# ahuang73/HemoCell

Measured on AMD Instinct MI355X. Metric: MLUPS + cell-vertex updates/s, 256^3 pipeflow 10% Hct, higher is better.
Workload: dtype f64

## Files before the change

hemocell_amd/capi.py:

```python
import ctypes as C
import os
import subprocess

_HERE = os.path.dirname(os.path.abspath(__file__))
LIB_PATH = os.path.join(_HERE, "lib", "libhemocell_amd.so")

c_double_p = C.POINTER(C.c_double)
c_long_p = C.POINTER(C.c_long)
c_int_p = C.POINTER(C.c_int)


class HcError(RuntimeError):
    pass


class Params(C.Structure):
    _fields_ = [(n, C.c_double) for n in
                ("dx", "dt", "nu_p", "rho_p", "kBT_p", "tau", "nu_lbm", "dm", "df", "f_limit", "kBT_lbm")]


class Material(C.Structure):
    _fields_ = [("kLink", C.c_double), ("kArea", C.c_double), ("kVolume", C.c_double), ("kBend", C.c_double),
                ("eta_m", C.c_double), ("radius", C.c_double), ("min_triangles", C.c_int),
                ("aspect_ratio", C.c_double), ("inner_edges", c_long_p), ("n_inner", C.c_int)]


class WbcMaterial(C.Structure):
    _fields_ = [("kInnerRigid", C.c_double), ("kCytoskeleton", C.c_double), ("coreRadius", C.c_double),
                ("radius", C.c_double)]


class CellTypeSpec(C.Structure):
    _fields_ = [("model", C.c_int), ("shape", C.c_int), ("material", Material), ("wbc", C.POINTER(WbcMaterial)),
                ("kInnerLink", C.c_double), ("stl_path", C.c_char_p)]


VP = C.c_void_p
SIGNATURES = {
    "hc_last_error": (C.c_char_p, []),
    "hc_init": (C.c_int, [C.c_int]),
    "hc_device_count": (C.c_int, [c_int_p]),
    "hc_set_stream": (C.c_int, [VP]),
    "hc_synchronize": (C.c_int, []),
    "hc_fork": (C.c_int, []),
    "hc_route": (C.c_int, [C.c_int]),
    "hc_join": (C.c_int, []),
    "hc_side_stream": (C.c_int, [C.POINTER(VP)]),
    "hc_set_overlap": (C.c_int, [C.c_int]),
    "hc_comm_init_env": (C.c_int, []),
    "hc_comm_init": (C.c_int, [C.c_int, C.c_int, C.c_int, C.c_char_p, C.c_int, C.c_int, C.c_int]),
    "hc_comm_finalize": (C.c_int, []),
    "hc_comm_info": (C.c_int, [c_int_p, c_int_p, c_int_p]),
    "hc_comm_barrier": (C.c_int, []),
    "hc_comm_allreduce": (C.c_int, [c_double_p, C.c_int, C.c_int]),
    "hc_comm_bcast": (C.c_int, [VP, C.c_size_t, C.c_int]),
    "hc_comm_allgather": (C.c_int, [VP, C.c_size_t, VP]),
    "hc_comm_exchange_host": (C.c_int, [C.c_int, VP, C.c_size_t, VP, C.c_size_t, VP, C.c_size_t, VP, C.c_size_t]),
    "hc_slab_stats": (C.c_int, [VP, c_double_p, C.c_int]),
    "hcl_slab_refresh_halos": (C.c_int, [VP, C.c_int]),
    "hcp_slab_sync_placement": (C.c_int, [VP, c_long_p]),
    "hcp_set_envelope": (C.c_int, [VP, C.c_double, c_double_p]),
    "hcp_envelope": (C.c_int, [VP, c_double_p, c_long_p]),
    "hcp_set_deletion_mode": (C.c_int, [VP, C.c_int]),
    "hcp_delete_incomplete_cells": (C.c_int, [VP, c_long_p]),
    "hcp_deletion_counts": (C.c_int, [VP, c_long_p, c_long_p, c_long_p, c_long_p]),
    "hcp_download_alive": (C.c_int, [VP, VP]),
    "hc_profile_enable": (C.c_int, [C.c_int]),
    "hc_profile_read": (C.c_int, [C.c_char_p, c_double_p, c_long_p]),
    "hc_profile_reset": (C.c_int, []),
    "hc_build_tag": (C.c_char_p, []),
    "hc_measure_copy_bandwidth": (C.c_int, [C.c_size_t, C.c_int, c_double_p]),
    "hcl_node_counts": (C.c_int, [VP, c_long_p]),
    "hc_debug_ibm_per_vertex": (C.c_int, [C.c_int]),
    "hc_set_reproducible_spread": (C.c_int, [C.c_int]),
    "hc_debug_force_plane_padding": (C.c_int, [C.c_int]),
    "hcl_create": (C.c_int, [C.POINTER(VP), C.c_int, C.c_int, C.c_int, c_int_p, C.c_double, C.c_int, C.c_int, C.c_int]),
    "hcl_destroy": (C.c_int, [VP]),
    "hcl_set_mask": (C.c_int, [VP, VP]),
    "hcl_init_equilibrium": (C.c_int, [VP, C.c_double, c_double_p]),
    "hcl_set_body_force_regions": (C.c_int, [VP, C.c_int, C.POINTER(C.c_int), c_double_p]),
    "hcl_set_body_force": (C.c_int, [VP, c_double_p]),
    "hcl_set_wall_velocity": (C.c_int, [VP, C.c_int, c_double_p]),
    "hcl_collide_stream": (C.c_int, [VP, C.c_int]),
    "hcl_set_lees_edwards": (C.c_int, [VP, C.c_double, C.c_double]),
    "hcl_set_lees_edwards_displacement": (C.c_int, [VP, C.c_double, C.c_double]),
    "hcl_lees_edwards_apply": (C.c_int, [VP]),
    "hcl_lees_edwards_state": (C.c_int, [VP, c_double_p]),
    "hcl_open_boundary_add": (C.c_int, [VP, C.c_int, C.c_int, c_int_p, C.c_int, c_int_p]),
    "hcl_open_boundary_add_box": (C.c_int, [VP, C.c_int, C.c_int, c_int_p, c_int_p, c_int_p]),
    "hcl_open_boundary_add_axis": (C.c_int, [VP, C.c_int, C.c_int, C.c_int, c_int_p, C.c_int, c_int_p]),
    "hcl_open_boundary_add_box_axis": (C.c_int, [VP, C.c_int, C.c_int, C.c_int, c_int_p, c_int_p, c_int_p]),
    "hcl_open_boundary_axes": (C.c_int, [VP, c_int_p, C.c_int, c_int_p]),
    "hcl_open_boundary_clear": (C.c_int, [VP]),
    "hcl_open_boundary_slots": (C.c_int, [VP, c_int_p, C.c_int, c_int_p]),
    "hcl_open_boundary_set_velocity": (C.c_int, [VP, C.c_int, C.c_int, VP, C.c_int]),
    "hcl_open_boundary_set_density": (C.c_int, [VP, C.c_int, C.c_int, VP, C.c_int]),
    "hcl_open_boundary_values": (C.c_int, [VP, C.c_int, C.c_int, c_double_p]),
    "hcl_plane_velocity": (C.c_int, [VP, C.c_int, c_int_p, C.c_int, VP, C.c_int]),
    "hcl_collide_stream_part": (C.c_int, [VP, C.c_int]),
    "hcl_step_end": (C.c_int, [VP]),
    "hcl_download_populations": (C.c_int, [VP, c_double_p]),
    "hcl_upload_populations": (C.c_int, [VP, c_double_p]),
    "hcl_download_rho_u": (C.c_int, [VP, c_double_p, c_double_p]),
    "hcl_download_pi_neq": (C.c_int, [VP, c_double_p]),
    "hcl_download_ibm_force": (C.c_int, [VP, c_double_p]),
    "hcl_zero_ibm_force": (C.c_int, [VP]),
    "hcl_halo_doubles": (C.c_size_t, [VP, C.c_int]),
    "hcl_halo_pack": (C.c_int, [VP, C.c_int, C.c_int, VP]),
    "hcl_halo_unpack": (C.c_int, [VP, C.c_int, C.c_int, VP]),
    "hcl_halo_pack_next": (C.c_int, [VP, C.c_int, C.c_int, VP]),
    "hcl_face_velocity_pack": (C.c_int, [VP, C.c_int, VP]),
    "hcl_face_velocity_pack_both": (C.c_int, [VP, VP, VP]),
    "hcl_halo_pack_both": (C.c_int, [VP, VP, VP, C.c_int]),
    "hcl_halo_unpack_both": (C.c_int, [VP, VP, VP]),
    "hcl_zero_force_halos": (C.c_int, [VP]),
    "hcl_download_face_velocity": (C.c_int, [VP, C.c_int, c_double_p]),
    "hcl_dims": (C.c_int, [VP, c_int_p]),
    "hcl_mlups_bytes_per_node": (C.c_double, [VP]),
    "hc_params_base": (C.c_int, [C.POINTER(Params)] + [C.c_double] * 5),
    "hcp_celltype_create": (C.c_int, [C.POINTER(VP), C.c_int, C.c_int, C.POINTER(Params), C.POINTER(Material)]),
    "hcp_celltype_create_wbc": (C.c_int, [C.POINTER(VP), C.c_int, C.POINTER(Params), C.POINTER(Material),
                                          C.POINTER(WbcMaterial)]),
    "hcp_celltype_wbc_constants": (C.c_int, [VP, c_double_p]),
    "hcp_celltype_create_ex": (C.c_int, [C.POINTER(VP), C.POINTER(Params), C.POINTER(CellTypeSpec)]),
    "hcp_celltype_malaria_constants": (C.c_int, [VP, c_double_p]),
    "hcp_celltype_destroy": (C.c_int, [VP]),
    "hcp_celltype_sizes": (C.c_int, [VP, c_int_p]),
    "hcp_celltype_tables": (C.c_int, [VP, c_double_p, c_long_p, c_long_p, c_double_p, c_double_p, c_double_p,
                                      c_long_p, c_double_p, c_double_p]),
    "hcp_celltype_tables2": (C.c_int, [VP, c_long_p, c_long_p, c_long_p, c_double_p, c_int_p]),
    "hcp_create": (C.c_int, [C.POINTER(VP), VP, C.POINTER(Params)]),
    "hcp_destroy": (C.c_int, [VP]),
    "hcp_add_type": (C.c_int, [VP, VP, C.c_int, c_int_p]),
    "hcp_add_cell": (C.c_int, [VP, C.c_int, C.c_long, c_double_p, c_double_p, C.c_double, c_int_p]),
    "hcp_add_cell_unchecked": (C.c_int, [VP, C.c_int, C.c_long, c_double_p, c_double_p]),
    "hcp_counts": (C.c_int, [VP, c_long_p, c_long_p, c_long_p]),
    "hcp_type_range": (C.c_int, [VP, C.c_int, c_long_p, c_long_p]),
    "hcp_download": (C.c_int, [VP, C.c_int, c_double_p]),
    "hcp_upload": (C.c_int, [VP, C.c_int, c_double_p]),
    "hcp_download_cell_ids": (C.c_int, [VP, c_long_p]),
    "hcp_download_records": (C.c_int, [VP, C.c_void_p, C.c_long]),
    "hcp_upload_records": (C.c_int, [VP, C.c_void_p, C.c_long]),
    "hcp_add_vertex_force": (C.c_int, [VP, c_long_p, C.c_int, c_double_p]),
    "hcp_set_repulsion": (C.c_int, [VP, C.c_double, C.c_double, C.c_int]),
    "hcp_repulsion": (C.c_int, [VP]),
    "hcp_download_repulsion": (C.c_int, [VP, c_double_p]),
    "hcl_fluid_stats": (C.c_int, [VP, C.c_int, c_double_p, C.POINTER(C.c_long)]),
    "hcp_vertex_stats": (C.c_int, [VP, C.c_int, c_double_p, C.POINTER(C.c_long)]),
    "hcp_set_boundary_repulsion": (C.c_int, [VP, C.c_double, C.c_double, C.c_int]),
    "hcp_boundary_repulsion": (C.c_int, [VP]),
    "hcp_spread": (C.c_int, [VP, C.c_int]),
    "hcp_interpolate": (C.c_int, [VP]),
    "hcp_interpolate_cells": (C.c_int, [VP, C.c_int, c_int_p, C.c_int]),
    "hcp_advance": (C.c_int, [VP, C.c_int]),
    "hcp_mechanics": (C.c_int, [VP, C.c_long, C.c_int]),
    "hcp_mechanics_components": (C.c_int, [VP, C.c_int, c_double_p]),
    "hc_iterate": (C.c_int, [VP, VP, c_long_p, C.c_int, C.c_int, C.c_int, C.c_int]),
    "hcp_cell_extents": (C.c_int, [VP, C.c_int, c_double_p]),
# ... 44 lines not shown
```

hemocell_amd/csrc/lattice.hip:

```cpp
#include "common.h"
#include "comm.h"
#include <algorithm>
#include <type_traits>

using namespace hc;

namespace {

struct LatArgs {
  const double *fin;
  double *fout;
  const double *Fin;
  double *Fzero;
  const uint8_t *mask;
  int nx, ny, nz;
  int plane;
  long xs;
  long npad;
  long qs;
  int x_begin;
  int x_split, x_jump;
  int wrap_x, per_y, per_z;
  double omega;
  double bx, by, bz;
  const int *row_z0, *row_cum, *blk_row;
  int nblk;
  int ibm;
  const uint8_t *dirty_in, *dirty_zero; uint8_t epoch_in, epoch_zero;
  double wall_u[4][3];
  int x0, nx_global;
  BodyRegions reg;
};

struct OpenArgs : LatArgs {
  const int *ob_code;
  const double *ob_val;
};
template <bool OPEN> using Args = std::conditional_t<OPEN, OpenArgs, LatArgs>;

__device__ __forceinline__ void body_at(const LatArgs &a, int x, int y, int z, double &bx, double &by, double &bz) {
  bx = a.bx; by = a.by; bz = a.bz;
  if (a.reg.n) region_force(a.reg, a.x0 + x, y, z, bx, by, bz);
}

struct Nbr {
  long xm, xp;
  int ym, yp, zm, zp;
  bool ym_ok, yp_ok, zm_ok, zp_ok;
};

__device__ __forceinline__ Nbr neighbours(const LatArgs &a, int x, int y, int z) {
  Nbr n;
  n.xm = -a.xs; n.xp = a.xs;
  if (a.wrap_x) {
    if (x == 0) n.xm = (long)(a.nx - 1) * a.xs;
    if (x == a.nx - 1) n.xp = -(long)(a.nx - 1) * a.xs;
  }
  n.ym = -a.nz; n.yp = a.nz; n.ym_ok = n.yp_ok = true;
  if (y == 0) { if (a.per_y) n.ym = (a.ny - 1) * a.nz; else n.ym_ok = false; }
  if (y == a.ny - 1) { if (a.per_y) n.yp = -(a.ny - 1) * a.nz; else n.yp_ok = false; }
  n.zm = -1; n.zp = 1; n.zm_ok = n.zp_ok = true;
  if (z == 0) { if (a.per_z) n.zm = a.nz - 1; else n.zm_ok = false; }
  if (z == a.nz - 1) { if (a.per_z) n.zp = -(a.nz - 1); else n.zp_ok = false; }
  return n;
}

template <int CX, int CY, int CZ>
__device__ __forceinline__ long src_off(const Nbr &n, bool &ok) {
  long off = 0; ok = true;
  if (CX == 1) off += n.xm; else if (CX == -1) off += n.xp;
  if (CY == 1) { off += n.ym; ok = ok && n.ym_ok; } else if (CY == -1) { off += n.yp; ok = ok && n.yp_ok; }
  if (CZ == 1) { off += n.zm; ok = ok && n.zm_ok; } else if (CZ == -1) { off += n.zp; ok = ok && n.zp_ok; }
  return off;
}
template <int CX, int CY, int CZ>
__device__ __forceinline__ long dst_off(const Nbr &n, bool &ok) {
  long off = 0; ok = true;
  if (CX == 1) off += n.xp; else if (CX == -1) off += n.xm;
  if (CY == 1) { off += n.yp; ok = ok && n.yp_ok; } else if (CY == -1) { off += n.ym; ok = ok && n.ym_ok; }
  if (CZ == 1) { off += n.zp; ok = ok && n.zp_ok; } else if (CZ == -1) { off += n.zm; ok = ok && n.zm_ok; }
  return off;
}

#define FOR_Q(M)                                                                                     \
  M(0, 0, 0, 0) M(1, -1, 0, 0) M(2, 0, -1, 0) M(3, 0, 0, -1) M(4, -1, -1, 0) M(5, -1, 1, 0)          \
  M(6, -1, 0, -1) M(7, -1, 0, 1) M(8, 0, -1, -1) M(9, 0, -1, 1) M(10, 1, 0, 0) M(11, 0, 1, 0)        \
  M(12, 0, 0, 1) M(13, 1, 1, 0) M(14, 1, -1, 0) M(15, 1, 0, 1) M(16, 1, 0, -1) M(17, 0, 1, 1)        \
  M(18, 0, 1, -1)

__device__ __forceinline__ constexpr double tq(int q) { return q == 0 ? 1. / 3. : ((q >= 1 && q <= 3) || (q >= 10 && q <= 12)) ? 1. / 18. : 1. / 36.; }

__device__ __forceinline__ void pull(const double *__restrict__ fin, long npad, long node, const Nbr &n, double f[HC_Q]) {
#define M(Q, CX, CY, CZ)                                   \
  {                                                        \
    bool ok; long off = src_off<CX, CY, CZ>(n, ok);        \
    f[Q] = ok ? fin[(long)Q * npad + node + off] : 0.0;    \
  }
  FOR_Q(M)
#undef M
}

template <bool OPEN>
__device__ __forceinline__ void complete_open(const Args<OPEN> &a, long node, double f[HC_Q]) {
  if constexpr (OPEN) {
    if (a.mask[node] == 0) {
      const int code = a.ob_code[node];
      if (code >= 0) zou_he_node(f, code, a.ob_val);
    }
  }
}

__device__ __forceinline__ void moments(const double f[HC_Q], double &rhoBar, double &jx, double &jy, double &jz) {
  double r = 0.0, x = 0.0, y = 0.0, z = 0.0;
#define M(Q, CX, CY, CZ)              \
  r += f[Q];                          \
  if (CX == 1) x += f[Q]; else if (CX == -1) x += -f[Q]; \
  if (CY == 1) y += f[Q]; else if (CY == -1) y += -f[Q]; \
  if (CZ == 1) z += f[Q]; else if (CZ == -1) z += -f[Q];
  FOR_Q(M)
#undef M
  rhoBar = r; jx = x; jy = y; jz = z;
}

template <int CX, int CY, int CZ>
__device__ __forceinline__ double cdot(double a0, double a1, double a2) {
  double s = 0.0; bool first = true;
  if (CX != 0) { s = (CX == 1 ? a0 : -a0); first = false; }
  if (CY != 0) { double t = (CY == 1 ? a1 : -a1); s = first ? t : s + t; first = false; }
  if (CZ != 0) { double t = (CZ == 1 ? a2 : -a2); s = first ? t : s + t; first = false; }
  return s;
}

__device__ __forceinline__ void collide_guo(double f[HC_Q], double Fx, double Fy, double Fz, double omega) {
  double rhoBar, j0, j1, j2;
  moments(f, rhoBar, j0, j1, j2);
  const double invRho = 1.0 / (1.0 + rhoBar);
  const double rho = 1.0 + rhoBar;
  const double u0 = j0 * invRho + Fx / 2.0, u1 = j1 * invRho + Fy / 2.0, u2 = j2 * invRho + Fz / 2.0;
  j0 = rho * u0; j1 = rho * u1; j2 = rho * u2;
  const double jSqr = j0 * j0 + j1 * j1 + j2 * j2;
  const double one_m_omega = 1.0 - omega;
  const double guo = 1.0 - omega / 2.0;
#define M(Q, CX, CY, CZ)                                                                     \
  {                                                                                          \
    const double c_j = cdot<CX, CY, CZ>(j0, j1, j2);                                         \
    const double feq = tq(Q) * (rhoBar + 3.0 * c_j + invRho * (4.5 * c_j * c_j - 1.5 * jSqr)); \
    f[Q] *= one_m_omega;                                                                     \
    f[Q] += omega * feq;                                                                     \
  }
  FOR_Q(M)
#undef M
#define M(Q, CX, CY, CZ)                                                                     \
  {                                                                                          \
    double c_u = cdot<CX, CY, CZ>(u0, u1, u2);                                               \
    c_u *= 9.0;                                                                              \
    double ft = (((double)CX - u0) * 3.0 + c_u * (double)CX) * Fx;                           \
    ft += (((double)CY - u1) * 3.0 + c_u * (double)CY) * Fy;                                 \
    ft += (((double)CZ - u2) * 3.0 + c_u * (double)CZ) * Fz;                                 \
    ft *= tq(Q);                                                                             \
    ft *= guo;                                                                               \
    f[Q] += ft;                                                                              \
  }
  FOR_Q(M)
#undef M
}

template <bool REGIONS, bool OPEN = false>
__global__ __launch_bounds__(256) void collide_stream_kernel(Args<OPEN> a) {
  const int x = a.x_begin + (int)blockIdx.y + ((int)blockIdx.y >= a.x_split ? a.x_jump : 0);
  const int xp = x + HALO;
  const int t = blockIdx.x * 256 + threadIdx.x;
  const int *cum = a.row_cum + (long)xp * (a.ny + 1);
  if (t >= cum[a.ny]) return;
  int lo = a.blk_row[(long)xp * (a.nblk + 1) + blockIdx.x], hi = a.blk_row[(long)xp * (a.nblk + 1) + blockIdx.x + 1];
  while (lo < hi) { const int mid = (lo + hi + 1) >> 1; if (cum[mid] <= t) lo = mid; else hi = mid - 1; }
  const int y = lo, z = a.row_z0[(long)xp * a.ny + y] + (t - cum[y]);
  const int p = y * a.nz + z;
  const long node = (long)(x + HALO) * a.xs + p;
  const uint8_t m = a.mask[node];
  if (m == 2) return;
  const Nbr n = neighbours(a, x, y, z);
  const bool fdirty = a.ibm && m == 0 && a.dirty_in[node >> 4] == a.epoch_in;
  double F0 = 0.0, F1 = 0.0, F2 = 0.0;
  if (fdirty) { F0 = a.Fin[3 * node]; F1 = a.Fin[3 * node + 1]; F2 = a.Fin[3 * node + 2]; }
  double f[HC_Q];
  pull(a.fin, a.qs, node, n, f);
  const bool wall = m != 0;
  if (wall) {
#pragma unroll
    for (int i = 1; i <= 9; i++) { double t = f[i]; f[i] = f[i + 9]; f[i + 9] = t; }
    if (m >= 3) {
      const double w0 = a.wall_u[m - 3][0], w1 = a.wall_u[m - 3][1], w2 = a.wall_u[m - 3][2];
#define M(Q, CX, CY, CZ)                                                                  \
      if (Q != 0) {                                                                       \
        constexpr int O = Q <= 9 ? Q + 9 : Q - 9;                                         \
        const double c_u = (double)CX * w0 + (double)CY * w1 + (double)CZ * w2;           \
        f[O] = f[O] - 6.0 * tq(Q) * c_u;                                                  \
      }
      FOR_Q(M)
#undef M
    }
  } else {
    double bx = a.bx, by = a.by, bz = a.bz;
    if (REGIONS) region_force(a.reg, a.x0 + x, y, z, bx, by, bz);
    double Fx = bx, Fy = by, Fz = bz;
    if (fdirty) {
      Fx = bx + F0; Fy = by + F1; Fz = bz + F2;
    }
    if constexpr (OPEN) {
      const int code = a.ob_code[node];
      if (code >= 0) zou_he_node(f, code, a.ob_val);
    }
    collide_guo(f, Fx, Fy, Fz, a.omega);
  }
#pragma unroll
  for (int q = 0; q < HC_Q; q++) __builtin_nontemporal_store(f[q], &a.fout[(long)q * a.qs + node]);
  if (a.ibm && a.dirty_zero[node >> 4] == a.epoch_zero) { a.Fzero[3 * node] = 0.0; a.Fzero[3 * node + 1] = 0.0; a.Fzero[3 * node + 2] = 0.0; }
}

__global__ void init_eq_kernel(LatArgs a, double rhoBar, double j0, double j1, double j2) {
  const int p = blockIdx.x * 256 + threadIdx.x;
  if (p >= a.plane) return;
  const int x = a.x_begin + blockIdx.y;
  const int y = p / a.nz, z = p - y * a.nz;
  const long node = (long)(x + HALO) * a.xs + p;
  const Nbr n = neighbours(a, x, y, z);
  const double invRho = 1.0 / (1.0 + rhoBar);
  const double jSqr = j0 * j0 + j1 * j1 + j2 * j2;
#define M(Q, CX, CY, CZ)                                                                        \
  {                                                                                             \
    bool ok; long off = dst_off<CX, CY, CZ>(n, ok);                                             \
    double v = 0.0;                                                                             \
    if (ok && a.mask[node + off] == 0) {                                                        \
      const double c_j = cdot<CX, CY, CZ>(j0, j1, j2);                                          \
      v = tq(Q) * (rhoBar + 3.0 * c_j + invRho * (4.5 * c_j * c_j - 1.5 * jSqr));               \
    }                                                                                           \
    a.fout[(long)Q * a.qs + node] = v;                                                          \
  }
  FOR_Q(M)
#undef M
}

__global__ void download_kernel(LatArgs a, double *aos) {
  const int p = blockIdx.x * 256 + threadIdx.x;
  if (p >= a.plane) return;
  const int x = a.x_begin + blockIdx.y;
  const int y = p / a.nz, z = p - y * a.nz;
  const long node = (long)(x + HALO) * a.xs + p;
  const Nbr n = neighbours(a, x, y, z);
  double f[HC_Q];
  pull(a.fin, a.qs, node, n, f);
  const long o = ((long)x * a.plane + p) * HC_Q;
#pragma unroll
  for (int q = 0; q < HC_Q; q++) aos[o + q] = f[q];
}

__global__ void upload_kernel(LatArgs a, const double *aos, int lo_ok, int hi_ok) {
  const int p = blockIdx.x * 256 + threadIdx.x;
  if (p >= a.plane) return;
  const int x = a.x_begin + blockIdx.y;
  const int y = p / a.nz, z = p - y * a.nz;
  const long node = (long)(x + HALO) * a.xs + p;
  const long bulk = (long)x * a.plane + p;
  Nbr nl = neighbours(a, x, y, z);
  nl.xm = nl.xm / a.xs * a.plane; nl.xp = nl.xp / a.xs * a.plane;
#define M(Q, CX, CY, CZ)                                                                  \
  {                                                                                       \
    bool ok; long off = dst_off<CX, CY, CZ>(nl, ok);                                      \
     \
    if (!a.wrap_x && ((CX == 1 && x == a.nx - 1 && !hi_ok) || (CX == -1 && x == 0 && !lo_ok))) ok = false; \
    a.fout[(long)Q * a.qs + node] = ok ? aos[(bulk + off) * HC_Q + Q] : 0.0;            \
  }
  FOR_Q(M)
#undef M
}

template <bool OPEN = false>
__global__ void rho_u_kernel(Args<OPEN> a, double *rho, double *u) {
  const int p = blockIdx.x * 256 + threadIdx.x;
  if (p >= a.plane) return;
  const int x = a.x_begin + blockIdx.y;
  const int y = p / a.nz, z = p - y * a.nz;
  const long node = (long)(x + HALO) * a.xs + p;
  const Nbr n = neighbours(a, x, y, z);
  double f[HC_Q];
  pull(a.fin, a.qs, node, n, f);
  complete_open<OPEN>(a, node, f);
  double rhoBar, j0, j1, j2;
  moments(f, rhoBar, j0, j1, j2);
  const double invRho = 1.0 / (1.0 + rhoBar);
  const long o = (long)x * a.plane + p;
  rho[o] = 1.0 + rhoBar;
  double bx, by, bz;
  body_at(a, x, y, z, bx, by, bz);
  u[3 * o] = j0 * invRho + (bx + a.Fin[3 * node]) / 2.0;
  u[3 * o + 1] = j1 * invRho + (by + a.Fin[3 * node + 1]) / 2.0;
  u[3 * o + 2] = j2 * invRho + (bz + a.Fin[3 * node + 2]) / 2.0;
}

template <bool OPEN = false>
// ... 144 lines not shown
  const long s2 = top ? modp((long)floor(D + (double)x), a.nx) : modp((long)ceil(-D + (double)x), a.nx);
  double f1[HC_Q], f2[HC_Q];
  pull(a.fin, a.qs, (s1 + HALO) * a.xs + row, neighbours(a, (int)s1, y, z), f1);
  pull(a.fin, a.qs, (s2 + HALO) * a.xs + row, neighbours(a, (int)s2, y, z), f2);
  if (top) {
    f[3] = g * f1[3] + (1 - g) * f2[3];
    f[6] = g * f1[16] + (1 - g) * f2[16];
    f[8] = g * f1[8] + (1 - g) * f2[8];
    f[16] = g * f1[6] + (1 - g) * f2[6];
    f[18] = g * f1[18] + (1 - g) * f2[18];
  } else {
    f[7] = g * f1[15] + (1 - g) * f2[15];
    f[9] = g * f1[9] + (1 - g) * f2[9];
    f[12] = g * f1[12] + (1 - g) * f2[12];
    f[15] = g * f1[7] + (1 - g) * f2[7];
    f[17] = g * f1[17] + (1 - g) * f2[17];
  }
  double *o = buf + (long)(1 - top) * HC_Q * nxy + r;
#pragma unroll
  for (int q = 0; q < HC_Q; q++) o[(long)q * nxy] = f[q];
}

__global__ __launch_bounds__(256) void le_scatter_kernel(LatArgs a, const double *buf) {
  const long nxy = (long)a.nx * a.ny;
  const long t = (long)blockIdx.x * 256 + threadIdx.x;
  if (t >= 2 * nxy) return;
  const int top = t < nxy ? 1 : 0;
  const long r = top ? t : t - nxy;
  const int x = (int)(r / a.ny), y = (int)(r - (long)x * a.ny);
  const int z = top ? a.nz - 1 : 0;
  const long node = (long)(x + HALO) * a.xs + (long)y * a.nz + z;
  const Nbr n = neighbours(a, x, y, z);
  const double *in = buf + (long)(1 - top) * HC_Q * nxy + r;
#define M(Q, CX, CY, CZ)                                                       \
  {                                                                            \
    bool ok; const long off = src_off<CX, CY, CZ>(n, ok);                      \
    if (ok) a.fout[(long)Q * a.qs + node + off] = in[(long)Q * nxy];           \
  }
  FOR_Q(M)
#undef M
}

struct HaloArgs {
  double *f;
  double *buf;
  double *buf2; int n_first;
  long npad; long xs; int plane;
  int n;
  int pop[HC_Q + 5];
  int xp[HC_Q + 5];
  int to_buf;
};
__global__ void halo_copy_kernel(HaloArgs h) {
  const int p = blockIdx.x * 256 + threadIdx.x;
  if (p >= h.plane) return;
  const int e = blockIdx.y;
  const long li = (long)h.pop[e] * h.npad + (long)h.xp[e] * h.xs + p;
  double *b = e < h.n_first ? h.buf + (long)e * h.plane + p : h.buf2 + (long)(e - h.n_first) * h.plane + p;
  if (h.to_buf) *b = h.f[li]; else h.f[li] = *b;
}

__global__ void zero_force_halo_kernel(double *F, long xs, int plane, int nx) {
  const int e = blockIdx.x * 256 + threadIdx.x;
  if (e >= 3 * plane) return;
  const int w = blockIdx.y;
  const int xp = w < HALO ? w : nx + w;
  F[3 * (long)xp * xs + e] = 0.0;
}

LatArgs make_args(const hc_lattice *L) {
  LatArgs a;
  a.fin = L->f[L->cur]; a.fout = L->f[1 - L->cur];
  const int fprev = (L->fcur + 2) % 3;
  a.Fin = L->force[L->fcur]; a.Fzero = L->force[fprev];
  a.x_split = 0x7fffffff; a.x_jump = 0;
  a.mask = L->mask;
  a.nx = L->nx; a.ny = L->ny; a.nz = L->nz; a.plane = (int)L->plane; a.xs = (long)L->xs; a.npad = (long)L->npad; a.qs = (long)L->qstride;
  a.x_begin = 0;
  a.wrap_x = (L->n_slabs == 1 && L->periodic[0]) ? 1 : 0;
  a.per_y = L->periodic[1]; a.per_z = L->periodic[2];
  a.omega = L->omega; a.bx = L->body[0]; a.by = L->body[1]; a.bz = L->body[2];
  a.x0 = L->x0; a.nx_global = L->nx_global; a.reg = L->regions;
  a.row_z0 = L->row_z0; a.row_cum = L->row_cum; a.blk_row = L->blk_row; a.nblk = L->nblk;
  a.ibm = L->ibm;
  a.dirty_in = L->fdirty[L->fcur]; a.dirty_zero = L->fdirty[fprev]; a.epoch_in = L->fepoch[L->fcur]; a.epoch_zero = L->fepoch[fprev];
  for (int c = 0; c < 4; c++) for (int d = 0; d < 3; d++) a.wall_u[c][d] = L->wall_u[c][d];
  return a;
}

OpenArgs open_args(const hc_lattice *L, const LatArgs &a) {
  OpenArgs o;
  static_cast<LatArgs &>(o) = a;
  o.ob_code = L->ob_code; o.ob_val = L->ob_val;
  return o;
}

dim3 plane_grid(const hc_lattice *L, int nplanes) { return dim3((unsigned)((L->plane + 255) / 256), (unsigned)nplanes, 1); }

int ensure_scratch(hc_lattice *L, size_t doubles) {
  if (L->scratch_doubles >= doubles) return HC_OK;
  if (L->scratch) HC_HIP(hipFree(L->scratch));
  L->scratch = nullptr; L->scratch_doubles = 0;
  HC_HIP(hipMalloc((void **)&L->scratch, doubles * sizeof(double)));
  L->scratch_doubles = doubles;
  return HC_OK;
}

int rebuild_active_map(hc_lattice *L) {
  const int NX = L->nx + 2 * HALO, ny = L->ny, nz = L->nz;
  std::vector<int> z0((size_t)NX * ny), cum((size_t)NX * (ny + 1));
  int max_active = 0;
  for (int x = 0; x < NX; x++) {
    int c = 0;
    for (int y = 0; y < ny; y++) {
      const uint8_t *row = L->hmask.data() + (size_t)x * L->xs + (size_t)y * nz;
      int a = 0, b = nz;
      while (a < nz && row[a] == 2) a++;
      while (b > a && row[b - 1] == 2) b--;
      z0[(size_t)x * ny + y] = a;
      cum[(size_t)x * (ny + 1) + y] = c;
      c += b - a;
    }
    cum[(size_t)x * (ny + 1) + ny] = c;
    max_active = std::max(max_active, c);
  }
  if (max_active == 0) max_active = 1;
  const int nblk = (max_active + 255) / 256;
  std::vector<int> blk((size_t)NX * (nblk + 1));
  for (int x = 0; x < NX; x++) {
    const int *cx = cum.data() + (size_t)x * (ny + 1);
    int y = 0;
    for (int b = 0; b <= nblk; b++) {
      const long t = (long)b * 256;
      while (y + 1 < ny && cx[y + 1] <= t) y++;
      blk[(size_t)x * (nblk + 1) + b] = y;
    }
  }
  for (int **p : {&L->row_z0, &L->row_cum, &L->blk_row}) if (*p) { HC_HIP(hipFree(*p)); *p = nullptr; }
  HC_HIP(hipMalloc((void **)&L->row_z0, z0.size() * sizeof(int)));
  HC_HIP(hipMalloc((void **)&L->row_cum, cum.size() * sizeof(int)));
  HC_HIP(hipMalloc((void **)&L->blk_row, blk.size() * sizeof(int)));
  HC_HIP(hipMemcpy(L->row_z0, z0.data(), z0.size() * sizeof(int), hipMemcpyHostToDevice));
  HC_HIP(hipMemcpy(L->row_cum, cum.data(), cum.size() * sizeof(int), hipMemcpyHostToDevice));
  HC_HIP(hipMemcpy(L->blk_row, blk.data(), blk.size() * sizeof(int), hipMemcpyHostToDevice));
  L->nblk = nblk; L->max_active = max_active;
  return HC_OK;
}

int rebuild_wall_bricks(hc_lattice *L) {
  const int NX = L->nx + 2 * HALO, ny = L->ny, nz = L->nz;
  std::vector<uint8_t> flag((size_t)L->nbx * L->nby * L->nbz, 0);
  for (int bx = 0; bx < L->nbx; bx++)
    for (int by = 0; by < L->nby; by++)
      for (int bz = 0; bz < L->nbz; bz++) {
        bool near = false;
        if (!L->periodic[1] && (by == 0 || by == L->nby - 1)) near = true;
        if (!L->periodic[2] && (bz == 0 || bz == L->nbz - 1)) near = true;
        if (bx * 8 < HALO + 1 || bx * 8 + 7 >= L->nx + HALO - 1) near = true;
        for (int x = bx * 8; x < std::min(NX, bx * 8 + 8) && !near; x++)
          for (int y = by * 8; y < std::min(ny, by * 8 + 8) && !near; y++) {
            const uint8_t *row = L->hmask.data() + (size_t)x * L->xs + (size_t)y * nz;
            for (int z = bz * 8; z < std::min(nz, bz * 8 + 8); z++) if (row[z] != 0) { near = true; break; }
          }
        flag[((size_t)bx * L->nby + by) * L->nbz + bz] = near ? 1 : 0;
      }
  if (!L->wallbrick) HC_HIP(hipMalloc((void **)&L->wallbrick, flag.size()));
  HC_HIP(hipMemcpy(L->wallbrick, flag.data(), flag.size(), hipMemcpyHostToDevice));
  return HC_OK;
}

int launch_collide(hc_lattice *L, int x_begin, int nplanes, int x2 = 0, int n2 = 0) {
  if (nplanes + n2 <= 0) return HC_OK;
  LatArgs a = make_args(L);
  a.x_begin = x_begin;
  if (n2 > 0) { a.x_split = nplanes; a.x_jump = x2 - (x_begin + nplanes); }
  const unsigned ny = (unsigned)(nplanes + n2);
  const dim3 grid((unsigned)((L->max_active + 255) / 256), ny, 1);
  if (L->ob_n > 0) {
    const OpenArgs o = open_args(L, a);
    if (L->regions.n) hipLaunchKernelGGL((collide_stream_kernel<true, true>), grid, dim3(256), 0, hc::stream(), o);
    else hipLaunchKernelGGL((collide_stream_kernel<false, true>), grid, dim3(256), 0, hc::stream(), o);
  } else if (L->regions.n) hipLaunchKernelGGL(collide_stream_kernel<true>, grid, dim3(256), 0, hc::stream(), a);
  else hipLaunchKernelGGL(collide_stream_kernel<false>, grid, dim3(256), 0, hc::stream(), a);
  HC_HIP(hipGetLastError());
  return HC_OK;
}

int launch_lees_edwards(hc_lattice *L) {
  hc::ProfScope prof(hc::PK_LEES_EDWARDS);
  LatArgs a = make_args(L);
  a.fout = L->f[L->cur];
  const long nthreads = 2L * L->nx * L->ny;
  const dim3 grid((unsigned)((nthreads + 255) / 256));
  hipLaunchKernelGGL(le_gather_kernel, grid, dim3(256), 0, hc::stream(), a, L->le_buf, L->le_D, L->le_v_top, L->le_v_bottom);
  HC_HIP(hipGetLastError());
  hipLaunchKernelGGL(le_scatter_kernel, grid, dim3(256), 0, hc::stream(), a, (const double *)L->le_buf);
  HC_HIP(hipGetLastError());
  return HC_OK;
}

}

int hc::lees_edwards_step(hc_lattice *L) { return L->le_on ? launch_lees_edwards(L) : HC_OK; }

static bool le_layers_fluid(const hc_lattice *L, const uint8_t *mask, size_t xs) {
  const int zs[4] = {0, 1, L->nz - 2, L->nz - 1};
  for (int x = HALO; x < L->nx + HALO; x++)
    for (int y = 0; y < L->ny; y++)
      for (int k = 0; k < 4; k++)
        if (mask[(size_t)x * xs + (size_t)y * L->nz + zs[k]] != 0) return false;
  return true;
}

static int g_force_plane_padding = 0;

extern "C" {

int hc_debug_force_plane_padding(int on) { g_force_plane_padding = on > 0 ? 1 : (on < 0 ? -1 : 0); return HC_OK; }

int hcl_create(hc_lattice **out, int nx, int ny, int nz, const int periodic[3], double omega,
               int x0, int nx_global, int n_slabs) {
  HC_REQUIRE(out && periodic, "hcl_create: null pointer");
  HC_REQUIRE(nx >= 2 && ny >= 2 && nz >= 2, "hcl_create: every dimension must be >= 2");
  HC_REQUIRE(n_slabs >= 1 && nx_global >= nx && x0 >= 0 && x0 + nx <= nx_global, "hcl_create: inconsistent slab decomposition");
  HC_REQUIRE((long)ny * nz < (1L << 30) && (long)(nx + 2 * HALO) * (((long)ny + 8) * nz + 32) < (1L << 31), "hcl_create: slab too large for 32-bit plane indexing");
  HC_REQUIRE(omega > 0.0 && omega < 2.0, "hcl_create: omega must be in (0,2)");
  if (hc::stream() == nullptr) { hc::set_error("hcl_create: hc_init() has not been called"); return HC_ERR_STATE; }
  hc_lattice *L = new hc_lattice();
  L->nx = nx; L->ny = ny; L->nz = nz;
  for (int d = 0; d < 3; d++) L->periodic[d] = periodic[d] ? 1 : 0;
  L->x0 = x0; L->nx_global = nx_global; L->n_slabs = n_slabs;
  L->omega = omega;
  L->plane = (size_t)ny * nz;
  L->xs = (L->plane + 15) / 16 * 16;
  if (g_force_plane_padding > 0 || (g_force_plane_padding == 0 && ((L->plane * sizeof(double)) % (1u << 20)) == 0)) L->xs += (size_t)(8 * nz + 15) / 16 * 16;
  if (g_force_plane_padding < 0) L->xs = L->plane;
  L->npad = (size_t)(nx + 2 * HALO) * L->xs;
  L->qstride = L->npad + 16 * 129;
  L->cur = 0; L->fcur = 0; L->ibm = 0;
  L->body[0] = L->body[1] = L->body[2] = 0.0;
  L->regions.n = 0;
  for (int c = 0; c < 4; c++) for (int d = 0; d < 3; d++) L->wall_u[c][d] = 0.0;
  L->scratch = nullptr; L->scratch_doubles = 0;
  L->f[0] = L->f[1] = nullptr; L->mask = nullptr;
  for (int k = 0; k < 3; k++) { L->force[k] = nullptr; L->fdirty[k] = nullptr; }
  for (int k = 0; k < 2; k++) {
    HC_HIP(hipMalloc((void **)&L->f[k], L->qstride * HC_Q * sizeof(double)));
    HC_HIP(hipMemsetAsync(L->f[k], 0, L->qstride * HC_Q * sizeof(double), hc::stream()));
  }
  for (int k = 0; k < 3; k++) {
    HC_HIP(hipMalloc((void **)&L->force[k], L->npad * 3 * sizeof(double)));
    HC_HIP(hipMemsetAsync(L->force[k], 0, L->npad * 3 * sizeof(double), hc::stream()));
  }
  HC_HIP(hipMalloc((void **)&L->mask, L->npad));
  HC_HIP(hipMemsetAsync(L->mask, 0, L->npad, hc::stream()));
  for (int k = 0; k < 3; k++) {
    HC_HIP(hipMalloc((void **)&L->fdirty[k], L->npad / 16 + 1));
    HC_HIP(hipMemsetAsync(L->fdirty[k], 0, L->npad / 16 + 1, hc::stream()));
    L->fepoch[k] = 1;
  }
  L->hmask.assign(L->npad, 0);
  L->row_z0 = L->row_cum = L->blk_row = nullptr;
  L->wallbrick = nullptr; L->nbx = (nx + 2 * HALO + 7) / 8; L->nby = (ny + 7) / 8; L->nbz = (nz + 7) / 8;
  { int rc = rebuild_active_map(L); if (rc != HC_OK) return rc; }
  { int rc = rebuild_wall_bricks(L); if (rc != HC_OK) return rc; }
  HC_HIP(hipStreamSynchronize(hc::stream()));
  *out = L;
  return HC_OK;
}

int hcl_destroy(hc_lattice *L) {
  if (!L) return HC_OK;
  hcs::lattice_destroyed(L);
  hipStreamSynchronize(hc::stream());
  for (int k = 0; k < 2; k++) if (L->f[k]) hipFree(L->f[k]);
  for (int k = 0; k < 3; k++) { if (L->force[k]) hipFree(L->force[k]); if (L->fdirty[k]) hipFree(L->fdirty[k]); }
  if (L->mask) hipFree(L->mask);
  if (L->scratch) hipFree(L->scratch);
  if (L->row_z0) hipFree(L->row_z0);
  if (L->row_cum) hipFree(L->row_cum);
  if (L->blk_row) hipFree(L->blk_row);
  if (L->wallbrick) hipFree(L->wallbrick);
  if (L->le_buf) hipFree(L->le_buf);
  if (L->ob_code) hipFree(L->ob_code);
  if (L->ob_val) hipFree(L->ob_val);
  if (L->ob_list) hipFree(L->ob_list);
  if (L->ob_out) hipFree(L->ob_out);
  delete L;
  return HC_OK;
}

int hcl_dims(const hc_lattice *L, int dims[3]) {
  HC_REQUIRE(L && dims, "hcl_dims: null pointer");
  dims[0] = L->nx; dims[1] = L->ny; dims[2] = L->nz;
  return HC_OK;
}

int hcl_node_counts(const hc_lattice *L, long counts[3]) {
  HC_REQUIRE(L && counts, "hcl_node_counts: null pointer");
  long fluid = 0, active = 0;
  for (int x = 0; x < L->nx; x++)
// ... 517 lines not shown
```

include/hemocell_amd.h:

```cpp
#ifndef HEMOCELL_AMD_H
#define HEMOCELL_AMD_H

#include <stddef.h>
#include <stdint.h>

#ifdef __cplusplus
extern "C" {
#endif

#define HC_OK 0
#define HC_ERR_HIP 1
#define HC_ERR_ARG 2
#define HC_ERR_STATE 3

#define HC_Q 19

typedef struct hc_lattice hc_lattice;
typedef struct hc_celltype hc_celltype;
typedef struct hc_cells hc_cells;

const char *hc_last_error(void);
int hc_init(int device);
int hc_device_count(int *count);
int hc_set_stream(void *hip_stream);
int hc_synchronize(void);
int hc_fork(void);
int hc_route(int side);
int hc_join(void);
int hc_side_stream(void **hip_stream);
int hc_set_overlap(int on);
int hc_profile_enable(int on);
int hc_profile_read(const char *kernel, double *total_ms, long *launches);
int hc_profile_reset(void);
const char *hc_build_tag(void);
int hc_measure_copy_bandwidth(size_t bytes, int repeats, double *gbytes_per_s);
int hc_set_reproducible_spread(int on);
int hc_debug_ibm_per_vertex(int on);
int hc_debug_force_plane_padding(int on);

#define HC_TRANSPORT_NONE 0
#define HC_TRANSPORT_RCCL 1
#define HC_TRANSPORT_TCP 2
#define HC_TRANSPORT_AUTO 3
int hc_comm_init_env(void);
int hc_comm_init(int rank, int world, int local_rank, const char *master_addr, int port, int transport, int init_device);
int hc_comm_finalize(void);
int hc_comm_info(int *rank, int *world, int *transport);
int hc_comm_barrier(void);
int hc_comm_allreduce(double *v, int n, int op);
int hc_comm_bcast(void *buf, size_t bytes, int root);
int hc_comm_allgather(const void *mine, size_t bytes, void *all);
int hc_comm_exchange_host(int periodic, const void *send_lo, size_t n_lo, const void *send_hi, size_t n_hi,
                          void *recv_lo, size_t m_lo, void *recv_hi, size_t m_hi);
int hc_slab_stats(hc_lattice *L, double out[8], int reset);

int hcl_create(hc_lattice **out, int nx, int ny, int nz, const int periodic[3], double omega,
               int x0, int nx_global, int n_slabs);
int hcl_destroy(hc_lattice *L);
int hcl_set_mask(hc_lattice *L, const uint8_t *mask_with_halo);
int hcl_init_equilibrium(hc_lattice *L, double rho, const double u[3]);
int hcl_set_body_force(hc_lattice *L, const double F[3]);
#define HC_MAX_FORCE_REGIONS 4
int hcl_set_body_force_regions(hc_lattice *L, int n, const int *boxes, const double *forces);
int hcl_set_wall_velocity(hc_lattice *L, int wall_class, const double u[3]);
int hcl_collide_stream(hc_lattice *L, int nsteps);
int hcl_set_lees_edwards(hc_lattice *L, double v_top, double v_bottom);
int hcl_set_lees_edwards_displacement(hc_lattice *L, double D, double d_per_iteration);
int hcl_lees_edwards_apply(hc_lattice *L);
int hcl_lees_edwards_state(const hc_lattice *L, double out[4]);
#define HC_OB_VELOCITY 0
#define HC_OB_PRESSURE 1
int hcl_open_boundary_add(hc_lattice *L, int kind, int orientation, const int *nodes, int n, int *first_slot);
int hcl_open_boundary_add_box(hc_lattice *L, int kind, int orientation, const int box[6], int *first_slot, int *n_nodes);
int hcl_open_boundary_add_axis(hc_lattice *L, int kind, int axis, int orientation, const int *nodes, int n, int *first_slot);
int hcl_open_boundary_add_box_axis(hc_lattice *L, int kind, int axis, int orientation, const int box[6], int *first_slot, int *n_nodes);
int hcl_open_boundary_clear(hc_lattice *L);
int hcl_open_boundary_slots(const hc_lattice *L, const int *nodes, int n, int *slots);
int hcl_open_boundary_axes(const hc_lattice *L, const int *nodes, int n, int *axes);
int hcl_open_boundary_set_velocity(hc_lattice *L, int first_slot, int n, const double *u, int on_device);
int hcl_open_boundary_set_density(hc_lattice *L, int first_slot, int n, const double *rho, int on_device);
int hcl_open_boundary_values(hc_lattice *L, int first_slot, int n, double *out);
int hcl_plane_velocity(hc_lattice *L, int x, const int *yz, int n, double *out, int on_device);
int hcl_slab_refresh_halos(hc_lattice *L, int width);
int hcl_collide_stream_part(hc_lattice *L, int part);
int hcl_zero_force_halos(hc_lattice *L);
int hcl_step_end(hc_lattice *L);
int hcl_download_populations(hc_lattice *L, double *f_aos);
int hcl_upload_populations(hc_lattice *L, const double *f_aos);
int hcl_download_rho_u(hc_lattice *L, double *rho, double *u);
int hcl_download_pi_neq(hc_lattice *L, double *pi);
int hcl_fluid_stats(hc_lattice *L, int what, double out[3], long *n_nodes);
int hcl_download_ibm_force(hc_lattice *L, double *F);
int hcl_zero_ibm_force(hc_lattice *L);
size_t hcl_halo_doubles(const hc_lattice *L, int width);
int hcl_halo_pack(hc_lattice *L, int side, int width, double *dev_buf);
int hcl_halo_unpack(hc_lattice *L, int side, int width, const double *dev_buf);
int hcl_halo_pack_next(hc_lattice *L, int side, int width, double *dev_buf);
int hcl_halo_pack_both(hc_lattice *L, double *dev_lo, double *dev_hi, int next);
int hcl_halo_unpack_both(hc_lattice *L, const double *dev_lo, const double *dev_hi);
int hcl_face_velocity_pack(hc_lattice *L, int side, double *dev_buf);
int hcl_face_velocity_pack_both(hc_lattice *L, double *dev_lo, double *dev_hi);
int hcl_download_face_velocity(hc_lattice *L, int side, double *host_u );
int hcl_dims(const hc_lattice *L, int dims[3]);
int hcl_node_counts(const hc_lattice *L, long counts[3]);
double hcl_mlups_bytes_per_node(const hc_lattice *L);

#define HC_MODEL_RBC_HO 0
#define HC_MODEL_PLT_SIMPLE 1
#define HC_MODEL_WBC_HO 2
#define HC_MODEL_RBC_MALARIA 3
#define HC_SHAPE_WBC_SPHERE 0
#define HC_SHAPE_RBC_FROM_SPHERE 1
#define HC_SHAPE_MESH_FROM_STL 2
#define HC_SHAPE_ELLIPSOID_FROM_SPHERE 6

typedef struct hc_params {
  double dx, dt, nu_p, rho_p, kBT_p;
  double tau, nu_lbm, dm, df, f_limit, kBT_lbm;
} hc_params;
int hc_params_base(hc_params *P, double dx, double dt, double nu_p, double rho_p, double kBT_p);

// ... 94 lines not shown
```

Baseline: 16750.

## Restructure collide-stream kernel into multi-chunk loop with software-prefetched row lookup

Rewrites the collide-stream kernel so each block can process several 256-node chunks in a loop. It prefetches the next chunk's row location and mask/dirty tags while the current chunk is pulled, using scheduling barriers and opaque asm to control instruction ordering. The default chunk count is 1, and a debug API lets the count be changed at runtime. With one chunk, the main change is a restructured single-iteration path with branchless tag loads, which may alter register use and scheduling.

```diff
diff --git a/hemocell_amd/capi.py b/hemocell_amd/capi.py
--- a/hemocell_amd/capi.py
+++ b/hemocell_amd/capi.py
@@ -74,6 +74,7 @@
     "hc_debug_ibm_per_vertex": (C.c_int, [C.c_int]),
     "hc_set_reproducible_spread": (C.c_int, [C.c_int]),
     "hc_debug_force_plane_padding": (C.c_int, [C.c_int]),
+    "hc_debug_collide_chunks": (C.c_int, [C.c_int]),
     "hcl_create": (C.c_int, [C.POINTER(VP), C.c_int, C.c_int, C.c_int, c_int_p, C.c_double, C.c_int, C.c_int, C.c_int]),
     "hcl_destroy": (C.c_int, [VP]),
     "hcl_set_mask": (C.c_int, [VP, VP]),
diff --git a/hemocell_amd/csrc/lattice.hip b/hemocell_amd/csrc/lattice.hip
--- a/hemocell_amd/csrc/lattice.hip
+++ b/hemocell_amd/csrc/lattice.hip
@@ -25,6 +25,7 @@
   double bx, by, bz;
   const int *row_z0, *row_cum, *blk_row;
   int nblk;
+  int chunks;
   int ibm;
   const uint8_t *dirty_in, *dirty_zero; uint8_t epoch_in, epoch_zero;
   double wall_u[4][3];
@@ -49,21 +50,22 @@
   bool ym_ok, yp_ok, zm_ok, zp_ok;
 };
 
-__device__ __forceinline__ Nbr neighbours(const LatArgs &a, int x, int y, int z) {
+__device__ __forceinline__ Nbr neighbours(const LatArgs &a, int ny, int nz, int x, int y, int z) {
   Nbr n;
   n.xm = -a.xs; n.xp = a.xs;
   if (a.wrap_x) {
     if (x == 0) n.xm = (long)(a.nx - 1) * a.xs;
     if (x == a.nx - 1) n.xp = -(long)(a.nx - 1) * a.xs;
   }
-  n.ym = -a.nz; n.yp = a.nz; n.ym_ok = n.yp_ok = true;
-  if (y == 0) { if (a.per_y) n.ym = (a.ny - 1) * a.nz; else n.ym_ok = false; }
-  if (y == a.ny - 1) { if (a.per_y) n.yp = -(a.ny - 1) * a.nz; else n.yp_ok = false; }
+  n.ym = -nz; n.yp = nz; n.ym_ok = n.yp_ok = true;
+  if (y == 0) { if (a.per_y) n.ym = (ny - 1) * nz; else n.ym_ok = false; }
+  if (y == ny - 1) { if (a.per_y) n.yp = -(ny - 1) * nz; else n.yp_ok = false; }
   n.zm = -1; n.zp = 1; n.zm_ok = n.zp_ok = true;
-  if (z == 0) { if (a.per_z) n.zm = a.nz - 1; else n.zm_ok = false; }
-  if (z == a.nz - 1) { if (a.per_z) n.zp = -(a.nz - 1); else n.zp_ok = false; }
+  if (z == 0) { if (a.per_z) n.zm = nz - 1; else n.zm_ok = false; }
+  if (z == nz - 1) { if (a.per_z) n.zp = -(nz - 1); else n.zp_ok = false; }
   return n;
 }
+__device__ __forceinline__ Nbr neighbours(const LatArgs &a, int x, int y, int z) { return neighbours(a, a.ny, a.nz, x, y, z); }
 
 template <int CX, int CY, int CZ>
 __device__ __forceinline__ long src_off(const Nbr &n, bool &ok) {
@@ -165,26 +167,30 @@
 #undef M
 }
 
-template <bool REGIONS, bool OPEN = false>
-__global__ __launch_bounds__(256) void collide_stream_kernel(Args<OPEN> a) {
-  const int x = a.x_begin + (int)blockIdx.y + ((int)blockIdx.y >= a.x_split ? a.x_jump : 0);
-  const int xp = x + HALO;
-  const int t = blockIdx.x * 256 + threadIdx.x;
-  const int *cum = a.row_cum + (long)xp * (a.ny + 1);
-  if (t >= cum[a.ny]) return;
-  int lo = a.blk_row[(long)xp * (a.nblk + 1) + blockIdx.x], hi = a.blk_row[(long)xp * (a.nblk + 1) + blockIdx.x + 1];
+struct Spot { int y, z; };
+struct Tags { unsigned m, din, dzero; };
+
+__device__ __forceinline__ Spot locate(const LatArgs &a, const int *cum, int xp, int chunk, int total) {
+  const int t = chunk * 256 + threadIdx.x;
+  const long b = (long)xp * (a.nblk + 1) + chunk;
+  int lo = a.blk_row[b], hi = a.blk_row[b + 1];
   while (lo < hi) { const int mid = (lo + hi + 1) >> 1; if (cum[mid] <= t) lo = mid; else hi = mid - 1; }
-  const int y = lo, z = a.row_z0[(long)xp * a.ny + y] + (t - cum[y]);
-  const int p = y * a.nz + z;
-  const long node = (long)(x + HALO) * a.xs + p;
-  const uint8_t m = a.mask[node];
-  if (m == 2) return;
-  const Nbr n = neighbours(a, x, y, z);
-  const bool fdirty = a.ibm && m == 0 && a.dirty_in[node >> 4] == a.epoch_in;
-  double F0 = 0.0, F1 = 0.0, F2 = 0.0;
-  if (fdirty) { F0 = a.Fin[3 * node]; F1 = a.Fin[3 * node + 1]; F2 = a.Fin[3 * node + 2]; }
-  double f[HC_Q];
-  pull(a.fin, a.qs, node, n, f);
+  Spot s;
+  s.y = lo; s.z = a.row_z0[(long)xp * a.ny + lo] + (t - cum[lo]);
+  if (t >= total) { s.y = -1; s.z = 0; }
+  return s;
+}
+
+__device__ __forceinline__ Tags tags_at(const LatArgs &a, long node) {
+  const uint8_t *din = a.ibm ? a.dirty_in : a.mask, *dzero = a.ibm ? a.dirty_zero : a.mask;
+  Tags g;
+  g.din = din[node >> 4]; g.dzero = dzero[node >> 4]; g.m = a.mask[node];
+  return g;
+}
+
+template <bool REGIONS, bool OPEN>
+__device__ __forceinline__ void process(const Args<OPEN> &a, long qs, double omega, int x, int y, int z, long node, unsigned m, bool fdirty, bool fzero,
+                                        double F0, double F1, double F2, double f[HC_Q]) {
   const bool wall = m != 0;
   if (wall) {
 #pragma unroll
@@ -211,11 +217,54 @@
       const int code = a.ob_code[node];
       if (code >= 0) zou_he_node(f, code, a.ob_val);
     }
-    collide_guo(f, Fx, Fy, Fz, a.omega);
+    collide_guo(f, Fx, Fy, Fz, omega);
   }
 #pragma unroll
-  for (int q = 0; q < HC_Q; q++) __builtin_nontemporal_store(f[q], &a.fout[(long)q * a.qs + node]);
-  if (a.ibm && a.dirty_zero[node >> 4] == a.epoch_zero) { a.Fzero[3 * node] = 0.0; a.Fzero[3 * node + 1] = 0.0; a.Fzero[3 * node + 2] = 0.0; }
+  for (int q = 0; q < HC_Q; q++) __builtin_nontemporal_store(f[q], &a.fout[(long)q * qs + node]);
+  if (fzero) { a.Fzero[3 * node] = 0.0; a.Fzero[3 * node + 1] = 0.0; a.Fzero[3 * node + 2] = 0.0; }
+}
+
+template <class T> __device__ __forceinline__ void opaque(T &v) { asm volatile("" : "+s"(v)); }
+
+template <bool REGIONS, bool OPEN = false>
+__global__ __launch_bounds__(256) void collide_stream_kernel(Args<OPEN> a) {
+  const int x = a.x_begin + (int)blockIdx.y + ((int)blockIdx.y >= a.x_split ? a.x_jump : 0);
+  const int xp = x + HALO;
+  const int *cum = a.row_cum + (long)xp * (a.ny + 1);
+  const int total = cum[a.ny];
+  int chunk = (int)blockIdx.x * a.chunks;
+  if (chunk * 256 >= total) return;
+  const long base = (long)xp * a.xs;
+  Spot s = locate(a, cum, xp, chunk, total);
+  Tags g = tags_at(a, base + (s.y < 0 ? 0 : s.y) * a.nz + s.z);
+  int left = a.chunks - 1;
+  if ((chunk + 1) * 256 >= total) left = 0;
+  Spot s1 = s;
+  if (left) s1 = locate(a, cum, xp, chunk + 1, total);
+  for (;;) {
+    long qs = a.qs; int ny = a.ny, nz = a.nz; double omega = a.omega;
+    opaque(qs); opaque(ny); opaque(nz); opaque(omega);
+    const bool live = s.y >= 0 && g.m != 2;
+    const int y = live ? s.y : 0, z = live ? s.z : 0;
+    const long node = base + y * nz + z;
+    const Nbr n = neighbours(a, ny, nz, x, y, z);
+    const bool fdirty = live && a.ibm && g.m == 0 && g.din == a.epoch_in;
+    const bool fzero = live && a.ibm && g.dzero == a.epoch_zero;
+    const unsigned m = g.m;
+    double F0 = 0.0, F1 = 0.0, F2 = 0.0;
+    if (fdirty) { F0 = a.Fin[3 * node]; F1 = a.Fin[3 * node + 1]; F2 = a.Fin[3 * node + 2]; }
+    double f[HC_Q];
+    pull(a.fin, qs, node, n, f);
+    g = tags_at(a, base + (s1.y < 0 ? 0 : s1.y) * nz + s1.z);
+    __builtin_amdgcn_sched_barrier(0);
+    if (live) process<REGIONS, OPEN>(a, qs, omega, x, y, z, node, m, fdirty, fzero, F0, F1, F2, f);
+    if (!left) break;
+    asm volatile("" : "+v"(g.m));
+    chunk++; left--;
+    if ((chunk + 1) * 256 >= total) left = 0;
+    s = s1;
+    if (left) s1 = locate(a, cum, xp, chunk + 1, total);
+  }
 }
 
 __global__ void init_eq_kernel(LatArgs a, double rhoBar, double j0, double j1, double j2) {
@@ -526,6 +575,7 @@
   a.omega = L->omega; a.bx = L->body[0]; a.by = L->body[1]; a.bz = L->body[2];
   a.x0 = L->x0; a.nx_global = L->nx_global; a.reg = L->regions;
   a.row_z0 = L->row_z0; a.row_cum = L->row_cum; a.blk_row = L->blk_row; a.nblk = L->nblk;
+  a.chunks = 1;
   a.ibm = L->ibm;
   a.dirty_in = L->fdirty[L->fcur]; a.dirty_zero = L->fdirty[fprev]; a.epoch_in = L->fepoch[L->fcur]; a.epoch_zero = L->fepoch[fprev];
   for (int c = 0; c < 4; c++) for (int d = 0; d < 3; d++) a.wall_u[c][d] = L->wall_u[c][d];
@@ -613,13 +663,18 @@
   return HC_OK;
 }
 
+constexpr int COLLIDE_CHUNKS = 1;
+int g_collide_chunks = 0;
+
 int launch_collide(hc_lattice *L, int x_begin, int nplanes, int x2 = 0, int n2 = 0) {
   if (nplanes + n2 <= 0) return HC_OK;
   LatArgs a = make_args(L);
   a.x_begin = x_begin;
   if (n2 > 0) { a.x_split = nplanes; a.x_jump = x2 - (x_begin + nplanes); }
   const unsigned ny = (unsigned)(nplanes + n2);
-  const dim3 grid((unsigned)((L->max_active + 255) / 256), ny, 1);
+  a.chunks = g_collide_chunks ? g_collide_chunks : COLLIDE_CHUNKS;
+  const int nchunk = (L->max_active + 255) / 256;
+  const dim3 grid((unsigned)((nchunk + a.chunks - 1) / a.chunks), ny, 1);
   if (L->ob_n > 0) {
     const OpenArgs o = open_args(L, a);
     if (L->regions.n) hipLaunchKernelGGL((collide_stream_kernel<true, true>), grid, dim3(256), 0, hc::stream(), o);
@@ -661,6 +716,12 @@
 extern "C" {
 
 int hc_debug_force_plane_padding(int on) { g_force_plane_padding = on > 0 ? 1 : (on < 0 ? -1 : 0); return HC_OK; }
+
+int hc_debug_collide_chunks(int k) {
+  HC_REQUIRE(k >= 0 && k <= 16, "hc_debug_collide_chunks: k must be 0 (default) or 1..16");
+  g_collide_chunks = k;
+  return HC_OK;
+}
 
 int hcl_create(hc_lattice **out, int nx, int ny, int nz, const int periodic[3], double omega,
                int x0, int nx_global, int n_slabs) {
diff --git a/include/hemocell_amd.h b/include/hemocell_amd.h
--- a/include/hemocell_amd.h
+++ b/include/hemocell_amd.h
@@ -37,6 +37,7 @@
 int hc_set_reproducible_spread(int on);
 int hc_debug_ibm_per_vertex(int on);
 int hc_debug_force_plane_padding(int on);
+int hc_debug_collide_chunks(int k);
 
 #define HC_TRANSPORT_NONE 0
 #define HC_TRANSPORT_RCCL 1
```

New measurement: 16720. Within noise of the previous version (-0.2%).
